# rbrito/deprecated-lame-mirror

Hardware: AMD Instinct MI355X
Metric: encoded audio seconds/sec (x real-time) at 44.1kHz stereo CBR128 (higher is better)
Workload: dtype f32

## Files before the change

### deprecated-lame-mirror_amd/csrc/lh_analysis.hip

```cpp
#include <stdint.h>
#include <math.h>

#ifdef LH_EMU
#include "hipemu.h"
#define LH_CONST static const
#else
#include <hip/hip_runtime.h>
#define LH_CONST __device__ static const
#endif

#if defined(LH_APROF) && !defined(LH_EMU)
__shared__ unsigned long long *lh_ap_base;
#define LH_PT(var) unsigned long long var = clock64()
#define LH_PA(idx, var) do { if (c.lane == 0) atomicAdd(&lh_ap_base[LH_NPROF * c.wave + 20 + (idx)], clock64() - var); } while (0)
#define LH_PC(idx) do { } while (0)
#endif
#define LH_CUSTOM_LDS "lh_lds_analysis.h"
#define LH_CUSTOM_SMP
#define LH_FZ_X(i) ((((i) >> 4) & 2) | (((i) >> 3) & 24) | (((i) >> 5) & 4))
#define LH_FZ(i) ((i) ^ LH_FZ_X(i))
#define LH_STAGE_IDX(i) LH_FZ(i)
#include "lh_static_tables.h"
#include "lh_dev_common.h"
#if !defined(LH_EMU)
#define LH_KRESTRICT __restrict__
#else
#define LH_KRESTRICT
#endif

#define LH_SPAN (lh_lds.work)
LH_DEVFN float
lh_smp(const LhCtx & c, int ch, int i)
{
    return LH_SPAN[ch * LH_BLKSIZE + LH_FZ(i)];
}

#include "lh_dev_psy_core.h"

struct LhGranuleAt {
    int     live;
    int     gr;
    long long at;
    long long frame_base;
};

LH_DEVFN LhGranuleAt
lh_granule_at(const LhStreamDesc & d, int g)
{
    LhGranuleAt o;
    int const nf = d.frame_end - d.frame_begin;
    int const fr = g / LH_NGR;
    o.live = g < LH_NGR * nf;
    o.gr = g - fr * LH_NGR;
    o.at = d.out_index + d.mid_rel + fr;
    o.frame_base = (long long) (576 * LH_NGR) * (d.frame_begin + fr) - LH_MF_START;
    return o;
}

LH_DEVFN LhStreamDesc
lh_desc_uniform(const LhStreamDesc * descs, int sidx)
{
    LhStreamDesc d = descs[sidx];
    d.pcm_l = lh_uni_ll(d.pcm_l);
    d.pcm_r = lh_uni_ll(d.pcm_r);
    d.pcm_base = lh_uni_ll(d.pcm_base);
    d.nsamples = lh_uni_ll(d.nsamples);
    d.out_index = lh_uni_ll(d.out_index);
    d.mid_rel = lh_uni_i(d.mid_rel);
    d.frame_begin = lh_uni_i(d.frame_begin);
    d.frame_end = lh_uni_i(d.frame_end);
    return d;
}

#ifdef LH_LSF
#define lh_attack_kernel lh_attack_kernel_lsf
#define lh_attack_scan_kernel lh_attack_scan_kernel_lsf
#define lh_analysis_kernel lh_analysis_kernel_lsf
#define lh_launch_analysis lh_launch_analysis_lsf
#define lh_emu_analysis lh_emu_analysis_lsf
#endif

#if defined(LH_APROF) && !defined(LH_EMU)
#define LH_AP_T0() unsigned long long ap_t = clock64()
#define LH_AP(k) do { unsigned long long const n_ = clock64(); if (c.lane == 0) atomicAdd(&aprof[64 * 0 + LH_NPROF * c.wave + (k)], n_ - ap_t); ap_t = n_; } while (0)
#else
#define LH_AP_T0() do { } while (0)
#define LH_AP(k) do { } while (0)
#endif
#define LH_FIR_SPAN 640

#ifndef LH_EMU
extern "C" __global__ void __launch_bounds__(64)
#else
void
#endif
lh_attack_kernel(const LhConfig * LH_KRESTRICT cfg, const int16_t * LH_KRESTRICT pcm, const float *pcmf, const LhStreamDesc * descs, LhMidFrame * frames,
                 int nstreams)
{
    __shared__ float span[2 * LH_FIR_SPAN];
    int const sidx = (int) blockIdx.y;
    LhCtx   c;
    c.cfg = cfg;
    c.T = nullptr;
    c.st = nullptr;
    c.pcm = pcm;
    c.pcmf = pcmf;
    c.d = lh_desc_uniform(descs, sidx);
    c.tid = (int) threadIdx.x;
    c.lane = c.tid;
    c.wave = 0;
    LhGranuleAt const ga = lh_granule_at(c.d, (int) blockIdx.x);
    if (!ga.live)
        return;
    int const lane = c.lane;
    int const n_chn_psy = (cfg->mode == LH_MODE_JOINT_STEREO) ? 4 : cfg->channels;
    int const bufbase = 576 + ga.gr * 576 - LH_FFTOFFSET;
    int const firbase = bufbase + 576 - 350 - LH_NSFIRLEN + 192;
    LhMidGr *mg = &frames[ga.at].small.gr[ga.gr];
    lh_stage_span < LH_FIR_SPAN, 64, 1 > (c, span, span + LH_FIR_SPAN, ga.frame_base + firbase);
    LH_WAVE_SYNC();
    {
        int const i0 = 9 * lane;
        float   x[2][30], y[2][9];
#pragma unroll
        for (int ch = 0; ch < 2; ch++)
#pragma unroll
            for (int t = 0; t < 30; t++)
                x[ch][t] = span[ch * LH_FIR_SPAN + i0 + t];
#pragma unroll
        for (int ch = 0; ch < 2; ch++)
#pragma unroll
            for (int m = 0; m < 9; m++) {
                float   sum1 = x[ch][m + 10], sum2 = 0.0;
#pragma unroll
                for (int j = 0; j < ((LH_NSFIRLEN - 1) / 2) - 1; j += 2) {
                    sum1 += lh_hp_fir[j] * (x[ch][m + j] + x[ch][m + LH_NSFIRLEN - j]);
                    sum2 += lh_hp_fir[j + 1] * (x[ch][m + j + 1] + x[ch][m + LH_NSFIRLEN - j - 1]);
                }
                y[ch][m] = sum1 + sum2;
            }
        LH_WAVE_SYNC();
#pragma unroll
        for (int ch = 0; ch < 2; ch++)
#pragma unroll
            for (int m = 0; m < 9; m++)
                span[ch * LH_FIR_SPAN + i0 + m] = y[ch][m];
    }
    LH_WAVE_SYNC();
    float   fl[9], fr[9];
#pragma unroll
    for (int k = 0; k < 9; k++) {
        fl[k] = span[lane + 64 * k];
        fr[k] = span[LH_FIR_SPAN + lane + 64 * k];
    }
    for (int chn = 0; chn < n_chn_psy; chn++) {
        uint32_t pk[8], pk8 = 0;
#pragma unroll
        for (int k = 0; k < 9; k++) {
            float const l = fl[k], r = fr[k];
            float const v = (chn == 0) ? l : (chn == 1) ? r : (chn == 2) ? l + r : l - r;
            if (k < 8)
                pk[k] = lh_f32_as_u32(lh_fabsf(v));
            else
                pk8 = lh_f32_as_u32(lh_fabsf(v));
        }
        {
            uint32_t const m8 = lh_wave_max8(pk);
            uint32_t const m9 = lh_wave_max_u32(pk8);
            if (lane < 9)
                mg->peak[chn][lane] = lh_u32_as_f32(lane == 8 ? m9 : m8);
        }
    }
}

#ifndef LH_SCAN_BLOCK
#define LH_SCAN_BLOCK 4
#endif
#ifndef LH_EMU
extern "C" __global__ void __launch_bounds__(64)
#else
void
#endif
lh_attack_scan_kernel(const LhConfig * LH_KRESTRICT cfg, const LhTables * LH_KRESTRICT T, const LhStreamDesc * descs, const LhStreamState * states,
                      LhMidFrame * frames, int nstreams)
{
    int const sidx = (int) blockIdx.x;
    int const lane = (int) threadIdx.x;
    LhStreamDesc const d = lh_desc_uniform(descs, sidx);
    int const nf = d.frame_end - d.frame_begin;
    if (nf <= 0)
        return;
    const LhStreamState *st = &states[sidx];
    int const n_chn_psy = lh_uni_i((cfg->mode == LH_MODE_JOINT_STEREO) ? 4 : cfg->channels);
    int const channels = lh_uni_i(cfg->channels), short_blocks = lh_uni_i(cfg->short_blocks);
    int const chn = lane >> 4, i = lane & 15, grp = lane & 48;
    int const mine = chn < n_chn_psy;
    float   le = st->last_en_subshort[chn][i < 9 ? i : 0];
    int     last_att = st->last_attacks[chn];
    float const thresh = T->attack_threshold[chn];
    int     bt_old0 = lh_uni_i(st->blocktype_old[0]), bt_old1 = lh_uni_i(st->blocktype_old[1]);
    int const ng = LH_NGR * nf;
    float   pk_blk[LH_SCAN_BLOCK];
#pragma unroll
    for (int j = 0; j < LH_SCAN_BLOCK; j++) {
        int const g = (j < ng) ? j : 0;
        pk_blk[j] = frames[d.out_index + d.mid_rel + g / LH_NGR].small.gr[g % LH_NGR].peak[chn][i < 9 ? i : 0];
    }
    for (int g0 = 0; g0 < ng; g0 += LH_SCAN_BLOCK) {
        float   pk_cur[LH_SCAN_BLOCK], ssf_blk[LH_SCAN_BLOCK];
        int     nsa_blk[LH_SCAN_BLOCK][4];
#pragma unroll
        for (int j = 0; j < LH_SCAN_BLOCK; j++) {
            int const gn = g0 + LH_SCAN_BLOCK + j, g = (gn < ng) ? gn : 0;
            pk_cur[j] = pk_blk[j];
            pk_blk[j] = frames[d.out_index + d.mid_rel + g / LH_NGR].small.gr[g % LH_NGR].peak[chn][i < 9 ? i : 0];
        }
#pragma unroll
        for (int j = 0; j < LH_SCAN_BLOCK; j++) {
            float const pk = pk_cur[j];
            float const fresh = pk < 1.0f ? 1.0f : pk;
            float const old = lh_shfl_f32(le, grp + ((i + 6) & 15)), older = lh_shfl_f32(le, grp + ((i + 4) & 15));
            float const got = lh_shfl_f32(fresh, grp + ((i - 3) & 15));
            float const e = (i < 3) ? old : got;
            float const e1 = lh_shfl_f32(e, grp + ((i - 1) & 15)), e0 = lh_shfl_f32(e, grp + ((i - 2) & 15));
            float const then = (i < 3) ? older : e0;
            float const ai = (i < 3) ? e / then : (e > then) ? e / then : (then > e * 10.0f) ? then / (e * 10.0f) : 0.0f;
            float const whole = e0 + e1 + e;
            int const tail_low = e * 6 < whole, mid_low = e1 * 6 < whole;
            uint64_t const over_all = lh_ballot(i < 12 && ai > thresh);
            unsigned const over = (unsigned) (over_all >> (16 * chn)) & 0xfffu;
            float   en_short[4];
            en_short[0] = lh_shfl_f32(whole, grp + 2);
            en_short[1] = lh_shfl_f32(whole, grp + 5);
            en_short[2] = lh_shfl_f32(whole, grp + 8);
            en_short[3] = lh_shfl_f32(whole, grp + 11);
            ssf_blk[j] = tail_low ? (mid_low ? 0.25f : 0.5f) : 1.0f;
            int    *nsa = nsa_blk[j];
            le = fresh;
            for (int gq = 0; gq < 4; gq++) {
                unsigned const bits = (over >> (3 * gq)) & 7u;
                nsa[gq] = bits ? ((bits & 1u) ? 1 : (bits & 2u) ? 2 : 3) : 0;
            }
            for (int q = 1; q < 4; q++) {
                float const u = en_short[q - 1];
                float const v = en_short[q];
                float const m = (u > v) ? u : v;
                if (m < 40000) {
                    if (u < 1.7f * v && v < 1.7f * u) {
                        if (q == 1 && nsa[0] <= nsa[q])
                            nsa[0] = 0;
                        nsa[q] = 0;
                    }
                }
            }
        }
#pragma unroll
        for (int j = 0; j < LH_SCAN_BLOCK; j++) {
            int const g = g0 + j;
            if (g >= ng)
                break;
            int const fr = g / LH_NGR, gr = g - fr * LH_NGR;
            LhMidGr *mg = &frames[d.out_index + d.mid_rel + fr].small.gr[gr];
            int    *nsa = nsa_blk[j];
            float const ssf = ssf_blk[j];
            int     uselong = 1;
            if (nsa[0] <= last_att)
                nsa[0] = 0;
            if (last_att == 3 || nsa[0] + nsa[1] + nsa[2] + nsa[3]) {
                uselong = 0;
                if (nsa[1] && nsa[0])
                    nsa[1] = 0;
                if (nsa[2] && nsa[1])
                    nsa[2] = 0;
                if (nsa[3] && nsa[2])
                    nsa[3] = 0;
            }
            if (!mine) {
                nsa[0] = nsa[1] = nsa[2] = nsa[3] = 0;
                uselong = 1;
            }
            else
                last_att = nsa[2];
            if (i == 5 || i == 8 || i == 11)
                mg->sub_short_factor[chn][(i - 5) / 3] = mine ? ssf : 1.0f;
            if (i < 4)
                mg->ns_attacks[chn][i] = (int8_t) (i == 0 ? nsa[0] : i == 1 ? nsa[1] : i == 2 ? nsa[2] : nsa[3]);
            {
                uint64_t const shorts = lh_ballot(!uselong);
                int const s0 = (int) (shorts & 1u), s1 = (int) ((shorts >> 16) & 1u), s23 = (int) ((shorts >> 32) & 0x10001u) != 0;
                int     ul0 = !s0, ul1 = (channels == 2) ? !s1 : 1;
                int     btd[2];
                if (s23)
                    ul0 = ul1 = 0;
                if (short_blocks == 1 && !(ul0 && ul1))
                    ul0 = ul1 = 0;
                if (short_blocks == 2)
                    ul0 = ul1 = 1;
                if (short_blocks == 3)
                    ul0 = ul1 = 0;
                for (int ch = 0; ch < 2; ch++) {
                    int     blocktype = LH_NORM_TYPE;
                    int     was = ch ? bt_old1 : bt_old0;
                    if (ch ? ul1 : ul0) {
                        if (was == LH_SHORT_TYPE)
                            blocktype = LH_STOP_TYPE;
                    }
                    else {
                        blocktype = LH_SHORT_TYPE;
                        if (was == LH_NORM_TYPE)
                            was = LH_START_TYPE;
                        if (was == LH_STOP_TYPE)
                            was = LH_SHORT_TYPE;
                    }
                    btd[ch] = was;
                    if (ch)
                        bt_old1 = lh_uni_i(blocktype);
                    else
                        bt_old0 = lh_uni_i(blocktype);
                }
                if (lane < 2) {
                    mg->uselong[lane] = (int8_t) (lane ? ul1 : ul0);
                    mg->block_type[lane] = (int8_t) (lane ? btd[1] : btd[0]);
                }
            }
        }
    }
}

template < int K1 > LH_DEVFN void
lh_fht_unit_fz(lh_f32x4 tw, float *fz, int u)
{
    constexpr int kx = K1 >> 1, k2 = K1 << 1, k3 = k2 + K1, k4 = k2 << 1;
    int const blk = u / kx, i = u - blk * kx;
    int const axis = (i == 0);
    int const lo = blk * k4 + i;
    int const hi = blk * k4 + (axis ? kx : K1 - i);
    int     al[4], ah[4];
    if (K1 == 4) {
        int const x = LH_FZ_X(lo);
#pragma unroll
        for (int j = 0; j < 4; j++) {
            al[j] = (lo + j * K1) ^ x;
            ah[j] = (hi + j * K1) ^ x;
        }
    }
    else if (K1 == 16) {
        int const x = LH_FZ_X(blk * k4);
#pragma unroll
        for (int j = 0; j < 4; j++) {
            al[j] = (lo + j * K1) ^ x ^ (j >= 2 ? 2 : 0);
            ah[j] = (hi + j * K1) ^ x ^ (j >= 2 ? 2 : 0);
        }
    }
    else if (K1 == 64) {
#pragma unroll
        for (int j = 0; j < 4; j++) {
            al[j] = (lo + j * K1) ^ LH_FZ_X(64 * j);
            ah[j] = (hi + j * K1) ^ (2 ^ LH_FZ_X(64 * j));
        }
    }
    else {
        int const xl = LH_FZ_X(lo), xh = LH_FZ_X(hi);
#pragma unroll
        for (int j = 0; j < 4; j++) {
            al[j] = (lo + j * K1) ^ xl;
            ah[j] = (hi + j * K1) ^ xh;
        }
    }
    float const p0 = fz[al[0]], p1 = fz[al[1]], p2 = fz[al[2]], p3 = fz[al[3]];
    float const q0 = fz[ah[0]], q1 = fz[ah[1]], q2 = fz[ah[2]], q3 = fz[ah[3]];
    float const s01 = p0 + p1, d01 = p0 - p1, s23 = p2 + p3, d23 = p2 - p3;
    float const r2 = (float) (LH_SQRT2 * q2), r3 = (float) (LH_SQRT2 * q3);
    float const t01 = q0 + q1, u01 = q0 - q1;
    float const a_l0 = s01 + s23, a_l1 = d01 + d23, a_l2 = s01 - s23, a_l3 = d01 - d23;
    float const a_h0 = t01 + r2, a_h1 = u01 + r3, a_h2 = t01 - r2, a_h3 = u01 - r3;
    LhRot const rq1 = lh_rot(tw.z, tw.w, p1, q1);
    LhRot const rq3 = lh_rot(tw.z, tw.w, p3, q3);
    float const le = p0 + rq1.along, lm = p0 - rq1.along;
    float const he = q0 + rq1.across, hm = q0 - rq1.across;
    float const l2e = p2 + rq3.along, l2m = p2 - rq3.along;
    float const h2e = q2 + rq3.across, h2m = q2 - rq3.across;
    LhRot const ra = lh_rot(tw.x, tw.y, l2e, h2m);
    LhRot const rb = lh_rot(tw.y, tw.x, h2e, l2m);
    fz[al[0]] = axis ? a_l0 : le + ra.along;
    fz[al[1]] = axis ? a_l1 : lm + rb.across;
    fz[al[2]] = axis ? a_l2 : le - ra.along;
    fz[al[3]] = axis ? a_l3 : lm - rb.across;
    fz[ah[0]] = axis ? a_h0 : he + rb.along;
    fz[ah[1]] = axis ? a_h1 : hm + ra.across;
    fz[ah[2]] = axis ? a_h2 : he - rb.along;
    fz[ah[3]] = axis ? a_h3 : hm - ra.across;
}

LH_DEVFN void
lh_fft_long_inplace(const LhCtx & c, float *x)
{
    const float *w = c.T->fft_window;
    int const lane = c.lane;
    float   o[2][8];
#pragma unroll
    for (int q = 0; q < 2; q++) {
        int const jj = lane + 64 * q;
        int const i = (int) lh_rev8((unsigned) jj);
        const float *xs = x + (i ^ LH_FZ_X(i));
        float   f0, f1, f2, f3, ww;
        f0 = w[i] * xs[0];
        ww = w[i + 0x200] * xs[0x200];
        f1 = f0 - ww;
        f0 = f0 + ww;
        f2 = w[i + 0x100] * xs[0x100];
        ww = w[i + 0x300] * xs[0x300];
        f3 = f2 - ww;
        f2 = f2 + ww;
        o[q][0] = f0 + f2;
        o[q][2] = f0 - f2;
        o[q][1] = f1 + f3;
        o[q][3] = f1 - f3;
        f0 = w[i + 0x001] * xs[0x001];
        ww = w[i + 0x201] * xs[0x201];
        f1 = f0 - ww;
        f0 = f0 + ww;
        f2 = w[i + 0x101] * xs[0x101];
        ww = w[i + 0x301] * xs[0x301];
        f3 = f2 - ww;
        f2 = f2 + ww;
        o[q][4] = f0 + f2;
        o[q][6] = f0 - f2;
        o[q][5] = f1 + f3;
        o[q][7] = f1 - f3;
    }
    {
        lh_f32x4 tw[4][2];
#pragma unroll
        for (int stage = 0; stage < 4; stage++) {
            int const kx = 2 << (2 * stage);
#pragma unroll
            for (int q = 0; q < 2; q++)
                tw[stage][q] = *(const lh_f32x4 *) c.T->fht_tw[stage][(lane + 64 * q) % kx];
        }
        LH_WAVE_SYNC_MEM();
#pragma unroll
        for (int q = 0; q < 2; q++) {
            int const at = 4 * (lane + 64 * q), xa = LH_FZ_X(at);
#pragma unroll
            for (int k = 0; k < 4; k++) {
                x[(at + k) ^ xa] = o[q][k];
                x[(at + k + LH_BLKSIZE / 2) ^ xa] = o[q][4 + k];
            }
        }
        LH_WAVE_SYNC_MEM();
#pragma unroll
        for (int q = 0; q < 2; q++)
            lh_fht_unit_fz < 4 > (tw[0][q], x, lane + 64 * q);
        LH_WAVE_SYNC_MEM();
#pragma unroll
        for (int q = 0; q < 2; q++)
            lh_fht_unit_fz < 16 > (tw[1][q], x, lane + 64 * q);
        LH_WAVE_SYNC_MEM();
#pragma unroll
        for (int q = 0; q < 2; q++)
            lh_fht_unit_fz < 64 > (tw[2][q], x, lane + 64 * q);
        LH_WAVE_SYNC_MEM();
#pragma unroll
        for (int q = 0; q < 2; q++)
            lh_fht_unit_fz < 256 > (tw[3][q], x, lane + 64 * q);
        LH_WAVE_SYNC_MEM();
    }
}

LH_DEVFN void
lh_fft_short_inplace(const LhCtx & c, float *x)
{
    const float *ws = c.T->fft_window_s;
    int const lane = c.lane;
    float   o[2][8];
#pragma unroll
    for (int q = 0; q < 2; q++) {
        int const t = lane + 64 * q, tt = t < 3 * (LH_BLKSIZE_S / 8) ? t : 0;
        int const b = tt >> 5, j = tt & 31;
        int const k = (576 / 3) * (b + 1);
        int const i = (int) lh_rev8((unsigned) (j << 2));
        float   f0, f1, f2, f3, w;
        f0 = ws[i] * x[LH_FZ(i + k)];
        w = ws[0x7f - i] * x[LH_FZ(i + k + 0x80)];
        f1 = f0 - w;
        f0 = f0 + w;
        f2 = ws[i + 0x40] * x[LH_FZ(i + k + 0x40)];
        w = ws[0x3f - i] * x[LH_FZ(i + k + 0xc0)];
        f3 = f2 - w;
        f2 = f2 + w;
        o[q][0] = f0 + f2;
        o[q][2] = f0 - f2;
        o[q][1] = f1 + f3;
        o[q][3] = f1 - f3;
        f0 = ws[i + 0x01] * x[LH_FZ(i + k + 0x01)];
        w = ws[0x7e - i] * x[LH_FZ(i + k + 0x81)];
        f1 = f0 - w;
        f0 = f0 + w;
        f2 = ws[i + 0x41] * x[LH_FZ(i + k + 0x41)];
        w = ws[0x3e - i] * x[LH_FZ(i + k + 0xc1)];
        f3 = f2 - w;
        f2 = f2 + w;
        o[q][4] = f0 + f2;
        o[q][6] = f0 - f2;
        o[q][5] = f1 + f3;
        o[q][7] = f1 - f3;
    }
    LH_WAVE_SYNC_MEM();
#pragma unroll
    for (int q = 0; q < 2; q++) {
        int const t = lane + 64 * q;
        if (t < 3 * (LH_BLKSIZE_S / 8)) {
            int const at = (t >> 5) * LH_BLKSIZE_S + 4 * (t & 31);
#pragma unroll
            for (int k = 0; k < 4; k++) {
                x[LH_FZ(at + k)] = o[q][k];
                x[LH_FZ(at + k + LH_BLKSIZE_S / 2)] = o[q][4 + k];
            }
        }
    }
    LH_WAVE_SYNC_MEM();
    for (int t = lane; t < 3 * (LH_BLKSIZE_S / 8); t += 64) {
        int const b = t >> 5, u = t & 31;
        lh_fht_unit_fz < 4 > (*(const lh_f32x4 *) c.T->fht_tw[0][u % 2], x + b * LH_BLKSIZE_S, u);
    }
    LH_WAVE_SYNC_MEM();
    for (int t = lane; t < 3 * (LH_BLKSIZE_S / 8); t += 64) {
        int const b = t >> 5, u = t & 31;
        lh_fht_unit_fz < 16 > (*(const lh_f32x4 *) c.T->fht_tw[1][u % 8], x + b * LH_BLKSIZE_S, u);
    }
    LH_WAVE_SYNC_MEM();
    for (int t = lane; t < 3 * (LH_BLKSIZE_S / 8); t += 64) {
        int const b = t >> 5, u = t & 31;
        lh_fht_unit_fz < 64 > (*(const lh_f32x4 *) c.T->fht_tw[2][u % 32], x + b * LH_BLKSIZE_S, u);
    }
    LH_WAVE_SYNC_MEM();
}

LH_DEVFN void
lh_an_spectra_short(const LhCtx & c, int w, int both, const float *wl, const float *wr, int first, float *out_own, float *out_ms)
{
    float const sqrt2_half = (float) (LH_SQRT2 * 0.5f);
    int const n = LH_BLKSIZE_S, h = n >> 1;
    for (int m = c.lane; m <= h; m += 64) {
        int const ire = first + m, iim = first + ((m == 0) ? 0 : (n - m));
        float const lre = wl[LH_FZ(ire)], lim = wl[LH_FZ(iim)], rre = wr[LH_FZ(ire)], rim = wr[LH_FZ(iim)];
        float const ore = w ? rre : lre, oim = w ? rim : lim;
        float const mre = (w ? lre - rre : lre + rre) * sqrt2_half, mim = (w ? lim - rim : lim + rim) * sqrt2_half;
        out_own[m] = (m == 0) ? ore * ore : (ore * ore + oim * oim) * 0.5f;
        if (both)
            out_ms[m] = (m == 0) ? mre * mre : (mre * mre + mim * mim) * 0.5f;
    }
}

LH_DEVFN void
lh_an_spectra(const LhCtx & c, int w, int own, int ms, float *work)
{
    float const sqrt2_half = (float) (LH_SQRT2 * 0.5f);
    const float *wl = work, *wr = work + LH_BLKSIZE;
    float   eo[9], em[9];
#pragma unroll
    for (int k = 0; k < 9; k++) {
        int const m0 = c.lane + 64 * k, m = m0 <= LH_BLKSIZE / 2 ? m0 : LH_BLKSIZE / 2;
        int const ire = m, iim = (m == 0) ? 0 : (LH_BLKSIZE - m);
        float const lre = wl[LH_FZ(ire)], lim = wl[LH_FZ(iim)], rre = wr[LH_FZ(ire)], rim = wr[LH_FZ(iim)];
        float const ore = w ? rre : lre, oim = w ? rim : lim;
        float const mre = (w ? lre - rre : lre + rre) * sqrt2_half, mim = (w ? lim - rim : lim + rim) * sqrt2_half;
        eo[k] = (m == 0) ? ore * ore : (ore * ore + oim * oim) * 0.5f;
        em[k] = (m == 0) ? mre * mre : (mre * mre + mim * mim) * 0.5f;
    }
    LH_SYNC_WG_LDS();
#pragma unroll
    for (int k = 0; k < 9; k++) {
        int const m = c.lane + 64 * k;
        if (m <= LH_BLKSIZE / 2) {
            if (own)
                work[w * LH_AN_ROW + m] = eo[k];
            if (ms)
                work[(w + 2) * LH_AN_ROW + m] = em[k];
        }
    }
}

#ifndef LH_EMU
extern "C" __global__ void __launch_bounds__(LH_NT, 6)
#else
void
#endif
lh_analysis_kernel(const LhConfig * LH_KRESTRICT cfg, const LhTables * LH_KRESTRICT T, const int16_t * LH_KRESTRICT pcm, const float *pcmf, const LhStreamDesc * descs,
                   LhMidFrame * frames, int nstreams, LhStreamState * states)
{
#if defined(LH_APROF) && !defined(LH_EMU)
    unsigned long long *aprof = &states[blockIdx.y].prof[0][0];
    if (threadIdx.x == 0)
        lh_ap_base = aprof;
#endif
    LH_AP_T0();
    LhLds & L = lh_lds;
    LhLds & P = L;
    float  *const work = L.work;
#define LH_AN_E(chn) (work + (chn) * LH_AN_ROW)
    int const sidx = (int) blockIdx.y;
    LhCtx   c;
    c.cfg = cfg;
    c.T = T;
    c.st = nullptr;
    c.pcm = pcm;
    c.pcmf = pcmf;
    c.d = lh_desc_uniform(descs, sidx);
    c.tid = (int) threadIdx.x;
    c.lane = c.tid & 63;
    c.wave = lh_uni_i(c.tid >> 6);
    LhGranuleAt const ga = lh_granule_at(c.d, (int) blockIdx.x);
    if (!ga.live)
        return;
    int const lane = c.lane, w = c.wave, gr = ga.gr;
    int const n_chn_psy = (cfg->mode == LH_MODE_JOINT_STEREO) ? 4 : cfg->channels;
    int const bufbase = 576 + gr * 576 - LH_FFTOFFSET;
    LhMidGr *mg = &frames[ga.at].small.gr[gr];
    if (c.tid < 2)
        L.uselong[c.tid] = mg->uselong[c.tid];
    LH_AP(0);
    lh_stage_span < LH_BLKSIZE, LH_NT > (c, LH_SPAN, LH_SPAN + LH_BLKSIZE, ga.frame_base + bufbase);
    LH_SYNC_WG_LDS();
    LH_AP(1);
    if (w < cfg->channels)
        lh_fft_long_inplace(c, work + w * LH_BLKSIZE);
    LH_SYNC_WG_LDS();
    LH_AP(2);
    lh_an_spectra(c, w, w < n_chn_psy, n_chn_psy == 4, work);
    LH_WAVE_SYNC_MEM();
    const float *stg_s3 = T->psy_l.s3;
    LH_WAVE_SYNC_MEM();
    LH_AP(3);
    LH_AP(4);
    {
        int const chn = (lane == 1) ? w + 2 : w;
        int const summing = lane < 3 && chn < n_chn_psy;
        int const loud = (lane == 2);
        float  *prod = (w == 0) ? P.eb : P.thr;
        const float *ew = T->ath_eql_w;
        const float *e = LH_AN_E(summing ? chn : w);
        float   acc = 0.0f;
        for (int h = 0; h < 2; h++) {
            int const j0 = 256 * h;
            LH_WAVE_SYNC_MEM();
#pragma unroll
            for (int q = 0; q < 4; q++) {
                int const j = j0 + lane + 64 * q;
                prod[j - j0] = LH_AN_E(w)[j] * ew[j];
            }
            LH_WAVE_SYNC_MEM();
            if (summing) {
                const lh_f32x4 *s4 = (const lh_f32x4 *) ((loud ? prod - j0 : e) + j0);
                lh_f32x4 a0 = s4[0], a1 = s4[1], a2 = s4[2], a3 = s4[3];
                if (h == 0 && !loud) {
                    a0.x = a0.y = a0.z = a0.w = 0.0f;
                    a1.x = a1.y = a1.z = a1.w = 0.0f;
                    a2.x = a2.y = a2.z = 0.0f;
                }
                for (int g = 0; g < 64; g += 4) {
                    int const n = (g + 4 < 64) ? g + 4 : g;
                    lh_f32x4 const b0 = s4[n], b1 = s4[n + 1], b2 = s4[n + 2], b3 = s4[n + 3];
#ifndef LH_EMU
                    asm volatile("v_add_f32 %0, %0, %1\n\tv_add_f32 %0, %0, %2\n\tv_add_f32 %0, %0, %3\n\tv_add_f32 %0, %0, %4\n\t"
                                 "v_add_f32 %0, %0, %5\n\tv_add_f32 %0, %0, %6\n\tv_add_f32 %0, %0, %7\n\tv_add_f32 %0, %0, %8\n\t"
                                 "v_add_f32 %0, %0, %9\n\tv_add_f32 %0, %0, %10\n\tv_add_f32 %0, %0, %11\n\tv_add_f32 %0, %0, %12\n\t"
                                 "v_add_f32 %0, %0, %13\n\tv_add_f32 %0, %0, %14\n\tv_add_f32 %0, %0, %15\n\tv_add_f32 %0, %0, %16"
                                 : "+v"(acc)
                                 : "v"(a0.x), "v"(a0.y), "v"(a0.z), "v"(a0.w), "v"(a1.x), "v"(a1.y), "v"(a1.z), "v"(a1.w),
                                   "v"(a2.x), "v"(a2.y), "v"(a2.z), "v"(a2.w), "v"(a3.x), "v"(a3.y), "v"(a3.z), "v"(a3.w));
#else
                    acc += a0.x; acc += a0.y; acc += a0.z; acc += a0.w;
                    acc += a1.x; acc += a1.y; acc += a1.z; acc += a1.w;
                    acc += a2.x; acc += a2.y; acc += a2.z; acc += a2.w;
                    acc += a3.x; acc += a3.y; acc += a3.z; acc += a3.w;
#endif
                    a0 = b0;
                    a1 = b1;
                    a2 = b2;
                    a3 = b3;
                }
            }
        }
        if (summing) {
            if (!loud) {
                acc += e[LH_BLKSIZE / 2];
                mg->tot_ener[chn] = acc;
            }
            else {
                acc = (float) (acc * LH_VO_SCALE);
                mg->loud[w] = acc;
            }
        }
        LH_WAVE_SYNC_MEM();
    }
    LH_SYNC_WG_LDS();
    LH_AP(5);
    {
        LhMidLong *ml = &frames[ga.at].lng;
        if (n_chn_psy == 4) {
            LhMaskChan const two[2] = {
                {w, LH_AN_E(w), &P.eb[w * 64], &P.thr[w * 64], nullptr, nullptr, &ml->m[gr][w]},
                {w + 2, LH_AN_E(w + 2), &P.eb[(w + 2) * 64], &P.thr[(w + 2) * 64], nullptr, nullptr, &ml->m[gr][w + 2]}
            };
            lh_compute_masking < 2, 1 > (c, 1, two, stg_s3);
        }
        else if (w < n_chn_psy) {
            LhMaskChan const one[1] = { {w, LH_AN_E(w), &P.eb[w * 64], &P.thr[w * 64], nullptr, nullptr, &ml->m[gr][w]} };
            lh_compute_masking < 1, 1 > (c, 1, one, stg_s3);
        }
    }
    LH_AP(6);
    int const any_short = lh_uni_i(!(L.uselong[0] && L.uselong[1]));
    if (!any_short)
        return;
    LH_SYNC_WG_LDS();
    lh_stage_span < LH_BLKSIZE, LH_NT > (c, LH_SPAN, LH_SPAN + LH_BLKSIZE, ga.frame_base + bufbase);
    LH_SYNC_WG_LDS();
    if (!L.uselong[w])
        lh_fft_short_inplace(c, work + w * LH_BLKSIZE);
    LH_SYNC_WG_LDS();
    for (int sblock = 0; sblock < 3; sblock++) {
        if (w < n_chn_psy && !L.uselong[w]) {
            LhMidShort *ms = &frames[ga.at].shrt;
            int const both = (n_chn_psy == 4);
            lh_an_spectra_short(c, w, both, work, work + LH_BLKSIZE, sblock * LH_BLKSIZE_S, L.eshort[w], L.eshort[w + 2 < 4 ? w + 2 : 3]);
            LH_WAVE_SYNC_MEM();
            if (both) {
                LhMaskChan const two[2] = {
                    {w, L.eshort[w], &P.eb[w * 64], &P.thr[w * 64], nullptr, nullptr, &ms->m[gr][sblock][w]},
                    {w + 2, L.eshort[w + 2], &P.eb[(w + 2) * 64], &P.thr[(w + 2) * 64], nullptr, nullptr, &ms->m[gr][sblock][w + 2]}
                };
                lh_compute_masking < 2, 1 > (c, 0, two, T->psy_s.s3);
            }
            else {
                LhMaskChan const one[1] = { {w, L.eshort[w], &P.eb[w * 64], &P.thr[w * 64], nullptr, nullptr, &ms->m[gr][sblock][w]} };
                lh_compute_masking < 1, 1 > (c, 0, one, T->psy_s.s3);
            }
        }
        LH_SYNC_WG_LDS();
    }
    LH_AP(7);
}

#ifndef LH_EMU
extern "C" int
lh_launch_analysis(const LhConfig * cfg, const LhTables * T, const int16_t * pcm, const float *pcmf, const LhStreamDesc * descs,
                   const LhStreamState * states, LhMidPools mid, int nstreams, int max_frames, void *stream)
{
    if (nstreams <= 0 || max_frames <= 0)
        return 0;
    dim3 const grid((unsigned) (LH_NGR * max_frames), (unsigned) nstreams);
    hipLaunchKernelGGL(lh_attack_kernel, grid, dim3(64), 0, (hipStream_t) stream, cfg, pcm, pcmf, descs, mid.frames, nstreams);
    hipLaunchKernelGGL(lh_attack_scan_kernel, dim3((unsigned) nstreams), dim3(64), 0, (hipStream_t) stream, cfg, T, descs, states,
                       mid.frames, nstreams);
    hipLaunchKernelGGL(lh_analysis_kernel, grid, dim3(LH_NT), 0, (hipStream_t) stream, cfg, T, pcm, pcmf, descs, mid.frames, nstreams,
                       (LhStreamState *) states);
    return (int) hipGetLastError();
}
#else
extern "C" int
lh_emu_analysis(const LhConfig * cfg, const LhTables * T, const int16_t * pcm, const float *pcmf, const LhStreamDesc * descs,
                const LhStreamState * states, const LhMidPools * pools, int nstreams, int max_frames)
{
    LhMidPools const mid = *pools;
    hipemu_dim3 grid = { (unsigned) (LH_NGR * max_frames), (unsigned) nstreams, 1 }, b64 = { 64, 1, 1 }, b128 = { LH_NT, 1, 1 };
    hipemu_dim3 grid1 = { (unsigned) nstreams, 1, 1 };
    hipemu_run(grid, b64,[=] () {
               lh_attack_kernel(cfg, pcm, pcmf, descs, mid.frames, nstreams);
               }
    );
    hipemu_run(grid1, b64,[=] () {
               lh_attack_scan_kernel(cfg, T, descs, states, mid.frames, nstreams);
               }
    );
    hipemu_run(grid, b128,[=] () {
               lh_analysis_kernel(cfg, T, pcm, pcmf, descs, mid.frames, nstreams, (LhStreamState *) states);
               }
    );
    return 0;
}
#endif
```

Before: 84120.

## Fuse attack FIR into analysis kernel and split short-block analysis into compacted kernel

```diff
diff --git a/deprecated-lame-mirror_amd/csrc/lh_analysis.hip b/deprecated-lame-mirror_amd/csrc/lh_analysis.hip
--- a/deprecated-lame-mirror_amd/csrc/lh_analysis.hip
+++ b/deprecated-lame-mirror_amd/csrc/lh_analysis.hip
@@ -73,7 +73,7 @@
 }
 
 #ifdef LH_LSF
-#define lh_attack_kernel lh_attack_kernel_lsf
+#define lh_analysis_short_kernel lh_analysis_short_kernel_lsf
 #define lh_attack_scan_kernel lh_attack_scan_kernel_lsf
 #define lh_analysis_kernel lh_analysis_kernel_lsf
 #define lh_launch_analysis lh_launch_analysis_lsf
@@ -87,73 +87,48 @@
 #define LH_AP_T0() do { } while (0)
 #define LH_AP(k) do { } while (0)
 #endif
-#define LH_FIR_SPAN 640
-
-#ifndef LH_EMU
-extern "C" __global__ void __launch_bounds__(64)
-#else
-void
-#endif
-lh_attack_kernel(const LhConfig * LH_KRESTRICT cfg, const int16_t * LH_KRESTRICT pcm, const float *pcmf, const LhStreamDesc * descs, LhMidFrame * frames,
-                 int nstreams)
-{
-    __shared__ float span[2 * LH_FIR_SPAN];
-    int const sidx = (int) blockIdx.y;
-    LhCtx   c;
-    c.cfg = cfg;
-    c.T = nullptr;
-    c.st = nullptr;
-    c.pcm = pcm;
-    c.pcmf = pcmf;
-    c.d = lh_desc_uniform(descs, sidx);
-    c.tid = (int) threadIdx.x;
-    c.lane = c.tid;
-    c.wave = 0;
-    LhGranuleAt const ga = lh_granule_at(c.d, (int) blockIdx.x);
-    if (!ga.live)
-        return;
-    int const lane = c.lane;
-    int const n_chn_psy = (cfg->mode == LH_MODE_JOINT_STEREO) ? 4 : cfg->channels;
-    int const bufbase = 576 + ga.gr * 576 - LH_FFTOFFSET;
-    int const firbase = bufbase + 576 - 350 - LH_NSFIRLEN + 192;
-    LhMidGr *mg = &frames[ga.at].small.gr[ga.gr];
-    lh_stage_span < LH_FIR_SPAN, 64, 1 > (c, span, span + LH_FIR_SPAN, ga.frame_base + firbase);
+#define LH_FIR_OFF (576 - 350 - LH_NSFIRLEN + 192)
+static_assert(LH_FIR_OFF + 9 * 63 + 8 + LH_NSFIRLEN < LH_BLKSIZE, "the filter's span lies inside the transforms'");
+LH_DEVFN void
+lh_an_attack_peaks(const LhCtx & c, float *work, int n_chn_psy, LhMidGr * mg)
+{
+    int const lane = c.lane, w = c.wave;
+    int const i0 = LH_FIR_OFF + 9 * lane;
+    float  *xs = work + w * LH_BLKSIZE;
+    float   x[30], y[9];
+#pragma unroll
+    for (int t = 0; t < 30; t++)
+        x[t] = xs[LH_FZ(i0 + t)];
+#pragma unroll
+    for (int m = 0; m < 9; m++) {
+        float   sum1 = x[m + 10], sum2 = 0.0;
+#pragma unroll
+        for (int j = 0; j < ((LH_NSFIRLEN - 1) / 2) - 1; j += 2) {
+            sum1 += lh_hp_fir[j] * (x[m + j] + x[m + LH_NSFIRLEN - j]);
+            sum2 += lh_hp_fir[j + 1] * (x[m + j + 1] + x[m + LH_NSFIRLEN - j - 1]);
+        }
+        y[m] = sum1 + sum2;
+    }
     LH_WAVE_SYNC();
-    {
-        int const i0 = 9 * lane;
-        float   x[2][30], y[2][9];
-#pragma unroll
-        for (int ch = 0; ch < 2; ch++)
-#pragma unroll
-            for (int t = 0; t < 30; t++)
-                x[ch][t] = span[ch * LH_FIR_SPAN + i0 + t];
-#pragma unroll
-        for (int ch = 0; ch < 2; ch++)
-#pragma unroll
-            for (int m = 0; m < 9; m++) {
-                float   sum1 = x[ch][m + 10], sum2 = 0.0;
-#pragma unroll
-                for (int j = 0; j < ((LH_NSFIRLEN - 1) / 2) - 1; j += 2) {
-                    sum1 += lh_hp_fir[j] * (x[ch][m + j] + x[ch][m + LH_NSFIRLEN - j]);
-                    sum2 += lh_hp_fir[j + 1] * (x[ch][m + j + 1] + x[ch][m + LH_NSFIRLEN - j - 1]);
-                }
-                y[ch][m] = sum1 + sum2;
-            }
-        LH_WAVE_SYNC();
-#pragma unroll
-        for (int ch = 0; ch < 2; ch++)
-#pragma unroll
-            for (int m = 0; m < 9; m++)
-                span[ch * LH_FIR_SPAN + i0 + m] = y[ch][m];
-    }
-    LH_WAVE_SYNC();
+#pragma unroll
+    for (int m = 0; m < 9; m++)
+        xs[LH_FZ(i0 + m)] = y[m];
+    LH_SYNC_WG_LDS();
     float   fl[9], fr[9];
 #pragma unroll
     for (int k = 0; k < 9; k++) {
-        fl[k] = span[lane + 64 * k];
-        fr[k] = span[LH_FIR_SPAN + lane + 64 * k];
-    }
-    for (int chn = 0; chn < n_chn_psy; chn++) {
+        fl[k] = work[LH_FZ(LH_FIR_OFF + lane + 64 * k)];
+        fr[k] = work[LH_BLKSIZE + LH_FZ(LH_FIR_OFF + lane + 64 * k)];
+    }
+    LH_SYNC_WG_LDS();
+#pragma unroll
+    for (int m = 0; m < 9; m++)
+        xs[LH_FZ(i0 + m)] = x[m];
+    LH_WAVE_SYNC_MEM();
+    for (int pass = 0; pass < 2; pass++) {
+        int const chn = w + 2 * pass;
+        if (chn >= n_chn_psy)
+            break;
         uint32_t pk[8], pk8 = 0;
 #pragma unroll
         for (int k = 0; k < 9; k++) {
@@ -618,12 +593,12 @@
     int const n_chn_psy = (cfg->mode == LH_MODE_JOINT_STEREO) ? 4 : cfg->channels;
     int const bufbase = 576 + gr * 576 - LH_FFTOFFSET;
     LhMidGr *mg = &frames[ga.at].small.gr[gr];
-    if (c.tid < 2)
-        L.uselong[c.tid] = mg->uselong[c.tid];
     LH_AP(0);
     lh_stage_span < LH_BLKSIZE, LH_NT > (c, LH_SPAN, LH_SPAN + LH_BLKSIZE, ga.frame_base + bufbase);
     LH_SYNC_WG_LDS();
     LH_AP(1);
+    lh_an_attack_peaks(c, work, n_chn_psy, mg);
+    LH_AP(13);
     if (w < cfg->channels)
         lh_fft_long_inplace(c, work + w * LH_BLKSIZE);
     LH_SYNC_WG_LDS();
@@ -712,34 +687,87 @@
         }
     }
     LH_AP(6);
-    int const any_short = lh_uni_i(!(L.uselong[0] && L.uselong[1]));
-    if (!any_short)
-        return;
-    LH_SYNC_WG_LDS();
-    lh_stage_span < LH_BLKSIZE, LH_NT > (c, LH_SPAN, LH_SPAN + LH_BLKSIZE, ga.frame_base + bufbase);
-    LH_SYNC_WG_LDS();
-    if (!L.uselong[w])
-        lh_fft_short_inplace(c, work + w * LH_BLKSIZE);
-    LH_SYNC_WG_LDS();
-    for (int sblock = 0; sblock < 3; sblock++) {
-        if (w < n_chn_psy && !L.uselong[w]) {
-            LhMidShort *ms = &frames[ga.at].shrt;
-            int const both = (n_chn_psy == 4);
-            lh_an_spectra_short(c, w, both, work, work + LH_BLKSIZE, sblock * LH_BLKSIZE_S, L.eshort[w], L.eshort[w + 2 < 4 ? w + 2 : 3]);
-            LH_WAVE_SYNC_MEM();
-            if (both) {
-                LhMaskChan const two[2] = {
-                    {w, L.eshort[w], &P.eb[w * 64], &P.thr[w * 64], nullptr, nullptr, &ms->m[gr][sblock][w]},
-                    {w + 2, L.eshort[w + 2], &P.eb[(w + 2) * 64], &P.thr[(w + 2) * 64], nullptr, nullptr, &ms->m[gr][sblock][w + 2]}
-                };
-                lh_compute_masking < 2, 1 > (c, 0, two, T->psy_s.s3);
-            }
-            else {
-                LhMaskChan const one[1] = { {w, L.eshort[w], &P.eb[w * 64], &P.thr[w * 64], nullptr, nullptr, &ms->m[gr][sblock][w]} };
-                lh_compute_masking < 1, 1 > (c, 0, one, T->psy_s.s3);
-            }
-        }
+}
+
+#define LH_AN_SRUN (64 / LH_NGR)
+#ifndef LH_EMU
+extern "C" __global__ void __launch_bounds__(LH_NT, 4)
+#else
+void
+#endif
+lh_analysis_short_kernel(const LhConfig * LH_KRESTRICT cfg, const LhTables * LH_KRESTRICT T, const int16_t * LH_KRESTRICT pcm, const float *pcmf,
+                         const LhStreamDesc * descs, LhMidFrame * frames, int nstreams, LhStreamState * states)
+{
+#if defined(LH_APROF) && !defined(LH_EMU)
+    unsigned long long *aprof = &states[blockIdx.y].prof[0][0];
+    if (threadIdx.x == 0)
+        lh_ap_base = aprof;
+#endif
+    LH_AP_T0();
+    LhLds & L = lh_lds;
+    LhLds & P = L;
+    float  *const work = L.work;
+    int const sidx = (int) blockIdx.y;
+    LhCtx   c;
+    c.cfg = cfg;
+    c.T = T;
+    c.st = nullptr;
+    c.pcm = pcm;
+    c.pcmf = pcmf;
+    c.d = lh_desc_uniform(descs, sidx);
+    c.tid = (int) threadIdx.x;
+    c.lane = c.tid & 63;
+    c.wave = lh_uni_i(c.tid >> 6);
+    int const lane = c.lane, w = c.wave;
+    int const n_chn_psy = (cfg->mode == LH_MODE_JOINT_STEREO) ? 4 : cfg->channels;
+    int const g0 = 64 * (int) blockIdx.x;
+    uint64_t short0, short1;
+    {
+        LhGranuleAt const ga = lh_granule_at(c.d, g0 + lane);
+        int     ul0 = 1, ul1 = 1;
+        if (ga.live) {
+            const LhMidGr *mg = &frames[ga.at].small.gr[ga.gr];
+            ul0 = mg->uselong[0];
+            ul1 = mg->uselong[1];
+        }
+        short0 = lh_ballot(!ul0);
+        short1 = lh_ballot(!ul1);
+    }
+    int     first = 1;
+    for (uint64_t todo = short0 | short1; todo; todo &= todo - 1) {
+        int const k = lh_uni_i(lh_ffs64(todo));
+        LhGranuleAt const ga = lh_granule_at(c.d, g0 + k);
+        int const gr = ga.gr;
+        int const bufbase = 576 + gr * 576 - LH_FFTOFFSET;
+        int const mine_long = !((w ? short1 : short0) >> k & 1);
+        if (!first)
+            LH_SYNC_WG_LDS();
+        first = 0;
+        lh_stage_span < LH_BLKSIZE, LH_NT > (c, LH_SPAN, LH_SPAN + LH_BLKSIZE, ga.frame_base + bufbase);
         LH_SYNC_WG_LDS();
+        if (!mine_long)
+            lh_fft_short_inplace(c, work + w * LH_BLKSIZE);
+        LH_SYNC_WG_LDS();
+        for (int sblock = 0; sblock < 3; sblock++) {
+            if (w < n_chn_psy && !mine_long) {
+                LhMidShort *ms = &frames[ga.at].shrt;
+                int const both = (n_chn_psy == 4);
+                lh_an_spectra_short(c, w, both, work, work + LH_BLKSIZE, sblock * LH_BLKSIZE_S, L.eshort[w], L.eshort[w + 2 < 4 ? w + 2 : 3]);
+                LH_WAVE_SYNC_MEM();
+                if (both) {
+                    LhMaskChan const two[2] = {
+                        {w, L.eshort[w], &P.eb[w * 64], &P.thr[w * 64], nullptr, nullptr, &ms->m[gr][sblock][w]},
+                        {w + 2, L.eshort[w + 2], &P.eb[(w + 2) * 64], &P.thr[(w + 2) * 64], nullptr, nullptr, &ms->m[gr][sblock][w + 2]}
+                    };
+                    lh_compute_masking < 2, 1 > (c, 0, two, T->psy_s.s3);
+                }
+                else {
+                    LhMaskChan const one[1] = { {w, L.eshort[w], &P.eb[w * 64], &P.thr[w * 64], nullptr, nullptr, &ms->m[gr][sblock][w]} };
+                    lh_compute_masking < 1, 1 > (c, 0, one, T->psy_s.s3);
+                }
+            }
+            LH_SYNC_WG_LDS();
+        }
     }
     LH_AP(7);
 }
@@ -752,10 +780,12 @@
     if (nstreams <= 0 || max_frames <= 0)
         return 0;
     dim3 const grid((unsigned) (LH_NGR * max_frames), (unsigned) nstreams);
-    hipLaunchKernelGGL(lh_attack_kernel, grid, dim3(64), 0, (hipStream_t) stream, cfg, pcm, pcmf, descs, mid.frames, nstreams);
+    dim3 const runs((unsigned) ((max_frames + LH_AN_SRUN - 1) / LH_AN_SRUN), (unsigned) nstreams);
+    hipLaunchKernelGGL(lh_analysis_kernel, grid, dim3(LH_NT), 0, (hipStream_t) stream, cfg, T, pcm, pcmf, descs, mid.frames, nstreams,
+                       (LhStreamState *) states);
     hipLaunchKernelGGL(lh_attack_scan_kernel, dim3((unsigned) nstreams), dim3(64), 0, (hipStream_t) stream, cfg, T, descs, states,
                        mid.frames, nstreams);
-    hipLaunchKernelGGL(lh_analysis_kernel, grid, dim3(LH_NT), 0, (hipStream_t) stream, cfg, T, pcm, pcmf, descs, mid.frames, nstreams,
+    hipLaunchKernelGGL(lh_analysis_short_kernel, runs, dim3(LH_NT), 0, (hipStream_t) stream, cfg, T, pcm, pcmf, descs, mid.frames, nstreams,
                        (LhStreamState *) states);
     return (int) hipGetLastError();
 }
@@ -767,16 +797,17 @@
     LhMidPools const mid = *pools;
     hipemu_dim3 grid = { (unsigned) (LH_NGR * max_frames), (unsigned) nstreams, 1 }, b64 = { 64, 1, 1 }, b128 = { LH_NT, 1, 1 };
     hipemu_dim3 grid1 = { (unsigned) nstreams, 1, 1 };
-    hipemu_run(grid, b64,[=] () {
-               lh_attack_kernel(cfg, pcm, pcmf, descs, mid.frames, nstreams);
+    hipemu_dim3 runs = { (unsigned) ((max_frames + LH_AN_SRUN - 1) / LH_AN_SRUN), (unsigned) nstreams, 1 };
+    hipemu_run(grid, b128,[=] () {
+               lh_analysis_kernel(cfg, T, pcm, pcmf, descs, mid.frames, nstreams, (LhStreamState *) states);
                }
     );
     hipemu_run(grid1, b64,[=] () {
                lh_attack_scan_kernel(cfg, T, descs, states, mid.frames, nstreams);
                }
     );
-    hipemu_run(grid, b128,[=] () {
-               lh_analysis_kernel(cfg, T, pcm, pcmf, descs, mid.frames, nstreams, (LhStreamState *) states);
+    hipemu_run(runs, b128,[=] () {
+               lh_analysis_short_kernel(cfg, T, pcm, pcmf, descs, mid.frames, nstreams, (LhStreamState *) states);
                }
     );
     return 0;
```

Result: no change. 83900 (-0.3%).
